# ai4ce/SNAC

Hardware: AMD Instinct MI355X
Metric: env-steps/sec at N=65536 envs (2D dynamic dense); bit-exact vs CPU (higher is better)
Workload: dtype f64; 1 GPU; 2D dynamic dense, 65536 envs/GPU, 600 vector steps/pass, uniform random actions (counter RNG), auto-reset, f64 obs of every step written; envs_per_gpu=65536, vector_steps_per_pass=600, env_steps_per_pass=39321600, parallelism=env-shard x1

## Files before the change

include/snac_hip.h:

```cpp
#ifndef SNAC_HIP_H
#define SNAC_HIP_H
#include <stddef.h>
#include <stdint.h>

#ifdef __cplusplus
extern "C" {
#endif

#define SNAC_ABI_VERSION 12

typedef enum snac_status {
    SNAC_OK = 0,
    SNAC_ERR_ARG = -1,
    SNAC_ERR_HIP = -2,
    SNAC_ERR_UNSUPPORTED = -3
} snac_status;

enum { SNAC_ENV_1D = 1, SNAC_ENV_2D = 2, SNAC_ENV_3D = 3 };
enum { SNAC_OBS_F64 = 0, SNAC_OBS_F32 = 1 };
enum { SNAC_OBS_NONE = 0, SNAC_OBS_ALL = 1, SNAC_OBS_LAST = 2, SNAC_OBS_TILED = 3 };
enum { SNAC_FLAG_NEED_RESET = 1 };
enum { SNAC_RULE_BRICK_GT = 1, SNAC_RULE_TIME_GT = 2 };
enum { SNAC_SCALARS_DEFAULT = 0, SNAC_SCALARS_RAW = 1, SNAC_SCALARS_NORM = 2 };
enum { SNAC_TAIL_POSITION = 1, SNAC_TAIL_PLAN = 2, SNAC_TAIL_RECORD = 4 };
// ... 104 lines not shown
typedef struct snac_rollout_record {
    int8_t* actions;
    int8_t* step_size;
    int16_t* plan_idx;
    uint8_t* first;
} snac_rollout_record;
int snac_rollout_rec(const snac_env_desc* desc, const snac_state* st, int32_t T, uint32_t t0, const int8_t* actions,
                     const int8_t* step_size, int obs_mode, void* obs, float* reward, uint8_t* done,
                     const snac_rollout_record* rec, void* stream);

int snac_rollout_tiled(const snac_env_desc* desc, const snac_state* st, int32_t T, uint32_t t0, const int8_t* actions,
                       const int8_t* step_size, int32_t ring_ticks, int32_t first_tick, void* obs, float* reward, uint8_t* done,
                       const snac_rollout_record* rec, void* stream);

int snac_replay_gather(const snac_env_desc* desc, const snac_state* st, int32_t cap, const void* obs_ring,
                       const uint8_t* first_ring, const int16_t* plan_idx_ring, const int32_t* tick_idx,
                       const int32_t* env_idx, int32_t batch, float* s_out, float* s_next_out, float* plan_out,
                       void* stream);
int snac_replay_gather_tiled(const snac_env_desc* desc, const snac_state* st, int32_t cap, const void* obs_ring,
                             const uint8_t* first_ring, const int16_t* plan_idx_ring, const int32_t* tick_idx,
                             const int32_t* env_idx, int32_t batch, float* s_out, float* s_next_out, float* plan_out,
                             void* stream);

int snac_make_plans(const snac_env_desc* desc, const snac_state* st, int32_t first, int32_t count, int32_t sparse,
                    uint64_t seed, int64_t plan_id_base, const int8_t* vertices, int32_t* area_out, void* stream);

int snac_plans_from_grids(const snac_env_desc* desc, const snac_state* st, int32_t m, int32_t first, const snac_state* src,
                          int32_t src_envs, const int32_t* src_rows, const double* environment_memory,
                          const int32_t* total_brick, void* stream);

int snac_observe(const snac_env_desc* desc, const snac_state* st, void* obs, void* stream);

int snac_iou(const snac_env_desc* desc, const snac_state* st, double* out, void* stream);

int snac_export_grid(const snac_env_desc* desc, const snac_state* st, double* out, void* stream);

typedef struct snac_mailbox snac_mailbox;
int snac_mailbox_create(const snac_env_desc* desc, uint32_t idle_us, snac_mailbox** out);
double* snac_mailbox_row(snac_mailbox* mb);
int snac_mailbox_touch(snac_mailbox* mb);
int snac_mailbox_step(snac_mailbox* mb, const snac_env_desc* desc, const snac_state* st, int32_t action, int32_t step_size);
int snac_mailbox_step_n(snac_mailbox* mb, const snac_env_desc* desc, const snac_state* st, const int8_t* actions, const int8_t* step_size);
float* snac_mailbox_reward(snac_mailbox* mb);
uint8_t* snac_mailbox_done(snac_mailbox* mb);
int snac_mailbox_settle(snac_mailbox* mb);
int snac_mailbox_quit(snac_mailbox* mb);
int snac_mailbox_destroy(snac_mailbox* mb);
int snac_mailbox_stats(const snac_mailbox* mb, uint32_t out[8]);

int snac_transition(const snac_env_desc* desc, const snac_state* st, int32_t m, const int32_t* src_index,
                    const int32_t* dst_index, uint32_t t, const int8_t* actions, const int8_t* step_size, void* obs,
                    float* reward, uint8_t* done, void* stream);

typedef struct snac_node2d {
    snac_env_hdr hdr;
    int32_t episode;
    int32_t zero0[3];
    uint32_t board[20];
    uint32_t zero1[4];
} snac_node2d;
int snac_nodes2d_pack(const snac_env_desc* desc, const snac_state* st, const int32_t* rows, int32_t m, snac_node2d* nodes, int32_t pool_rows,
                      const int32_t* node_rows, void* stream);
int snac_nodes2d_unpack(const snac_env_desc* desc, const snac_node2d* nodes, int32_t pool_rows, const int32_t* node_rows, int32_t m, snac_state* st,
                        const int32_t* rows, void* stream);
int snac_transition_nodes2d(const snac_env_desc* desc, const snac_state* st, snac_node2d* nodes, int32_t pool_rows, int32_t m,
                            const int32_t* src_index, const int32_t* dst_index, uint32_t t, const int8_t* actions, const int8_t* step_size,
// ... 120 lines not shown
```

snac_amd/_lib.py:

```python
import ctypes as C
import os
import subprocess

import numpy as np

HERE = os.path.dirname(os.path.abspath(__file__))
LIB_PATH = os.environ.get("SNAC_HIP_LIB") or os.path.join(HERE, "libsnac_hip.so")
CSRC = os.path.join(HERE, "csrc")
INCLUDE = os.path.join(os.path.dirname(HERE), "include")

SNAC_OK = 0
ABI_VERSION = 12
ENV_1D, ENV_2D, ENV_3D = 1, 2, 3
OBS_F64, OBS_F32 = 0, 1
OBS_NONE, OBS_ALL, OBS_LAST, OBS_TILED = 0, 1, 2, 3
FLAG_NEED_RESET = 1
RULE_BRICK_GT, RULE_TIME_GT = 1, 2
SCALARS_DEFAULT, SCALARS_RAW, SCALARS_NORM = 0, 1, 2
TAIL_POSITION, TAIL_PLAN, TAIL_RECORD = 1, 2, 4

EXPORTS = ("snac_version", "snac_last_error", "snac_env_sizes", "snac_obs_dim", "snac_reset", "snac_reset_scalar", "snac_step",
           "snac_step_scalar", "snac_rollout",
           "snac_rollout_rec", "snac_replay_gather", "snac_make_plans", "snac_observe", "snac_iou", "snac_export_grid", "snac_transition",
           "snac_import_state", "snac_obs_equal", "snac_discounted_return", "snac_plans_from_grids", "snac_mailbox_create", "snac_mailbox_row", "snac_mailbox_touch", "snac_mailbox_step", "snac_mailbox_step_n", "snac_mailbox_reward", "snac_mailbox_done",
           "snac_mailbox_quit", "snac_mailbox_settle", "snac_mailbox_destroy", "snac_mailbox_stats", "snac_stream_sync", "snac_rollout_tiled", "snac_replay_gather_tiled", "snac_traj_alloc",
           "snac_traj_alloc_ex", "snac_traj_free", "snac_traj_layout", "snac_traj_describe", "snac_traj_reserved_bytes", "snac_last_kernel", "snac_tuning",
           "snac_nodes2d_pack", "snac_nodes2d_unpack", "snac_transition_nodes2d", "snac_nodes1d_pack", "snac_nodes1d_unpack",
           "snac_transition_nodes1d", "snac_nodes3d_pack", "snac_nodes3d_unpack", "snac_transition_nodes3d",
           "snac_evaluate_nodes1d", "snac_evaluate_nodes2d", "snac_evaluate_nodes3d", "snac_action_dist", "snac_uct_select", "snac_uct_backup",
           "snac_uct_advance", "snac_uct_select_paths", "snac_uct_backup_paths", "snac_observe_nodes1d", "snac_observe_nodes2d",
           "snac_observe_nodes3d", "snac_uct_select_puct", "snac_uct_set_priors", "snac_uct_pick_moves", "snac_uct_restart",
           "snac_uct_returns", "snac_uct_select_paths_norm", "snac_uct_select_puct_norm", "snac_uct_backup_paths_norm", "snac_uct_bounds")


class Sizes(C.Structure):
    _fields_ = [(n, C.c_int32) for n in (
        "obs_dim", "num_actions", "total_step", "half_window", "env_height", "env_width", "plan_height", "plan_width",
        "grid_elems", "grid_elem_bytes", "plan_elems", "plan_elem_bytes")]


class EnvDesc(C.Structure):
    _fields_ = [("kind", C.c_int32), ("dynamic", C.c_int32), ("num_envs", C.c_int32), ("num_plans", C.c_int32),
                ("obs_dtype", C.c_int32), ("static_plan", C.c_int32), ("seed", C.c_uint64), ("env_id_base", C.c_int64),
                ("total_step", C.c_int32), ("rules", C.c_int32), ("frame_value", C.c_int32), ("obs_scalars", C.c_int32),
                ("obs_tail", C.c_int32), ("action_dist", C.c_int32)]


class RolloutRecord(C.Structure):
    _fields_ = [("actions", C.c_void_p), ("step_size", C.c_void_p), ("plan_idx", C.c_void_p), ("first", C.c_void_p)]


class State(C.Structure):
    _fields_ = [("hdr", C.c_void_p), ("episode", C.c_void_p), ("grid", C.c_void_p), ("plans", C.c_void_p),
                ("plan_tb", C.c_void_p), ("stat_episodes", C.c_void_p), ("stat_return", C.c_void_p),
                ("stat_iou_fx", C.c_void_p)]


TRAJ_INFO_WINDOWS = 64


class TrajInfo(C.Structure):
    _fields_ = ([(n, C.c_int32) for n in ("layout", "rebuilds", "pool_groups", "probe_launches", "windows", "windows_slow")]
                + [(n, C.c_float) for n in ("self_us_per_gib", "fast_us_per_gib", "slow_us_per_gib", "window_max_us_per_gib",
                                            "window_mean_us_per_gib", "block_us_per_gib", "build_ms")]
                + [("bytes", C.c_uint64), ("window_us", C.c_float * TRAJ_INFO_WINDOWS)])
# ... 26 lines not shown


def lib():
    global _lib
    if _lib is None:
        if not os.path.exists(LIB_PATH):
            raise SnacError("libsnac_hip.so is not built (%s); run __graft_entry__.build() or `make -C snac_amd/csrc`. "
                            "There is no CPU fallback." % LIB_PATH)
        import torch

        L = C.CDLL(LIB_PATH)
        vp = C.c_void_p
        L.snac_version.restype = C.c_int
        L.snac_last_error.restype = C.c_char_p
        L.snac_last_kernel.restype = C.c_char_p
        L.snac_stream_sync.argtypes = [vp]
        L.snac_env_sizes.argtypes = [C.c_int, C.c_int, C.POINTER(Sizes)]
        L.snac_obs_dim.argtypes = [C.POINTER(EnvDesc)]
        L.snac_reset.argtypes = [C.POINTER(EnvDesc), C.POINTER(State), vp, vp, vp, vp]
        L.snac_reset_scalar.argtypes = [C.POINTER(EnvDesc), C.POINTER(State), C.c_int32, vp, vp]
        L.snac_step_scalar.argtypes = [C.POINTER(EnvDesc), C.POINTER(State), C.c_uint32, C.c_int32, C.c_int32, C.c_int, vp, vp, vp, vp]
        L.snac_step.argtypes = [C.POINTER(EnvDesc), C.POINTER(State), C.c_uint32, vp, vp, C.c_int, vp, vp, vp, vp]
        L.snac_rollout.argtypes = [C.POINTER(EnvDesc), C.POINTER(State), C.c_int32, C.c_uint32, vp, vp, C.c_int, vp, vp, vp, vp]
        L.snac_rollout_rec.argtypes = [C.POINTER(EnvDesc), C.POINTER(State), C.c_int32, C.c_uint32, vp, vp, C.c_int, vp, vp, vp,
                                       C.POINTER(RolloutRecord), vp]
        L.snac_replay_gather.argtypes = [C.POINTER(EnvDesc), C.POINTER(State), C.c_int32, vp, vp, vp, vp, vp, C.c_int32, vp, vp, vp, vp]
        L.snac_replay_gather_tiled.argtypes = L.snac_replay_gather.argtypes
        L.snac_rollout_tiled.argtypes = [C.POINTER(EnvDesc), C.POINTER(State), C.c_int32, C.c_uint32, vp, vp, C.c_int32, C.c_int32, vp, vp, vp,
                                         C.POINTER(RolloutRecord), vp]
        L.snac_make_plans.argtypes = [C.POINTER(EnvDesc), C.POINTER(State), C.c_int32, C.c_int32, C.c_int32, C.c_uint64, C.c_int64, vp, vp, vp]
        L.snac_observe.argtypes = [C.POINTER(EnvDesc), C.POINTER(State), vp, vp]
        L.snac_iou.argtypes = [C.POINTER(EnvDesc), C.POINTER(State), vp, vp]
        L.snac_export_grid.argtypes = [C.POINTER(EnvDesc), C.POINTER(State), vp, vp]
        L.snac_transition.argtypes = [C.POINTER(EnvDesc), C.POINTER(State), C.c_int32, vp, vp, C.c_uint32, vp, vp, vp, vp, vp, vp]
        L.snac_nodes2d_pack.argtypes = [C.POINTER(EnvDesc), C.POINTER(State), vp, C.c_int32, vp, C.c_int32, vp, vp]
        L.snac_nodes2d_unpack.argtypes = [C.POINTER(EnvDesc), vp, C.c_int32, vp, C.c_int32, C.POINTER(State), vp, vp]
        L.snac_transition_nodes2d.argtypes = [C.POINTER(EnvDesc), C.POINTER(State), vp, C.c_int32, C.c_int32, vp, vp, C.c_uint32, vp, vp, vp, vp, vp, vp]
        for k in ("1d", "3d"):
            getattr(L, "snac_nodes%s_pack" % k).argtypes = L.snac_nodes2d_pack.argtypes
            getattr(L, "snac_nodes%s_unpack" % k).argtypes = L.snac_nodes2d_unpack.argtypes
            getattr(L, "snac_transition_nodes%s" % k).argtypes = L.snac_transition_nodes2d.argtypes
        L.snac_import_state.argtypes = [C.POINTER(EnvDesc), C.POINTER(State), C.c_int32, vp, vp, vp, vp, vp, vp, vp, vp]
        L.snac_plans_from_grids.argtypes = [C.POINTER(EnvDesc), C.POINTER(State), C.c_int32, C.c_int32, C.POINTER(State), C.c_int32, vp, vp, vp, vp]
        L.snac_mailbox_create.argtypes = [C.POINTER(EnvDesc), C.c_uint32, C.POINTER(vp)]
        L.snac_mailbox_row.argtypes, L.snac_mailbox_row.restype = [vp], vp
        L.snac_mailbox_reward.argtypes, L.snac_mailbox_reward.restype = [vp], vp
        L.snac_mailbox_done.argtypes, L.snac_mailbox_done.restype = [vp], vp
        L.snac_mailbox_step_n.argtypes = [vp, C.POINTER(EnvDesc), C.POINTER(State), vp, vp]
        L.snac_mailbox_touch.argtypes = [vp]
        L.snac_mailbox_step.argtypes = [vp, C.POINTER(EnvDesc), C.POINTER(State), C.c_int32, C.c_int32]
        L.snac_mailbox_quit.argtypes = [vp]
        L.snac_mailbox_settle.argtypes = [vp]
        L.snac_mailbox_destroy.argtypes = [vp]
        L.snac_mailbox_stats.argtypes = [vp, C.POINTER(C.c_uint32 * 8)]
        L.snac_obs_equal.argtypes = [C.POINTER(EnvDesc), vp, vp, C.c_int32, vp, vp, C.c_int32, C.c_int32, vp, vp]
        L.snac_discounted_return.argtypes = [C.c_int32, C.c_int32, vp, vp, vp, vp, vp, vp, vp]
        for k in ("1d", "2d", "3d"):
            getattr(L, "snac_evaluate_nodes%s" % k).argtypes = [C.POINTER(EnvDesc), C.POINTER(State), vp, C.c_int32, C.c_int32, vp, C.c_int32, C.c_uint32,
                                                                vp, vp, vp, vp]
        L.snac_action_dist.argtypes = [C.c_int32, C.POINTER(C.c_uint32), C.POINTER(C.c_int32)]
        L.snac_uct_select.argtypes = [C.c_int32, vp, C.c_int32, C.c_int32, C.c_int32, C.c_double, vp, vp, C.c_int32, vp, vp, vp, vp, vp, vp, vp, vp]
        L.snac_uct_backup.argtypes = [C.c_int32, vp, C.c_int32, C.c_int32, C.c_int32, C.c_double, vp, vp, vp, vp, vp, vp, vp, vp]
        L.snac_uct_advance.argtypes = [C.c_int32, vp, C.c_int32, C.c_int32, C.c_int32, vp, C.c_int32, C.c_int32, vp, vp, vp, vp, vp, vp, vp, vp]
        L.snac_uct_select_paths.argtypes = [C.c_int32, vp, C.c_int32, C.c_int32, C.c_int32, C.c_int32, C.c_double, C.c_double, vp, vp, C.c_int32,
                                            vp, vp, vp, vp, vp, vp, vp, vp, vp]
        L.snac_uct_backup_paths.argtypes = [C.c_int32, vp, C.c_int32, C.c_int32, C.c_int32, C.c_int32, C.c_double, vp, vp, vp, vp, vp, vp, vp, vp]
# ... 68 lines not shown
```

snac_amd/batched.py:

```python
import ctypes as C

import numpy as np
import torch

from . import _lib
from . import plans as _plans

_KINDS = {1: 1, 2: 2, 3: 3, "1d": 1, "2d": 2, "3d": 3, "1D": 1, "2D": 2, "3D": 3}
_GRID_DTYPE = {1: torch.int16, 2: torch.int32, 3: torch.int16}


def _ptr(t):
    return None if t is None else C.c_void_p(t.data_ptr())


_raw_stream = getattr(torch._C, "_cuda_getCurrentRawStream", None)
_current_device = getattr(torch._C, "_cuda_getDevice", None) or torch.cuda.current_device


def _meta(*tensors):
    return tuple(None if t is None else (t.shape, t.stride(), t.dtype) for t in tensors)


class BatchedDMPEnv:

    LAYOUTS = {None: {}, "lnet1d": dict(obs_tail=("position",)), "lnet2d": dict(frame_value=2, obs_scalars="norm"),
               "ppo": dict(obs_scalars="raw"), "ppo_plan": dict(obs_scalars="raw", obs_tail=("plan",))}
    _TAILS = {"position": _lib.TAIL_POSITION, "plan": _lib.TAIL_PLAN, "record": _lib.TAIL_RECORD}

    def __init__(self, kind, dynamic, num_envs, plans=None, plan_choose=0, density="dense", split="train",
                 device="cuda", seed=1, obs_dtype=torch.float64, env_id_base=0, total_step=None, plan_tb=None,
                 brick_gt=False, time_gt=False, layout=None, frame_value=None, obs_scalars=None, obs_tail=None, static_plan=0,
                 empty_plans=None, action_probs=None):
# ... 28 lines not shown
        if not isinstance(tail, int):
            tail = sum(self._TAILS[t] for t in set(tail))
        self.obs_tail = int(tail)
        self.total_step = int(total_step) if total_step else sz.total_step
        dev, N = self.device, self.num_envs
        if empty_plans is not None:
            P = int(empty_plans)
            if plans is not None or not 1 <= P <= 32767:
                raise ValueError("empty_plans: 1 .. 32767 rows, without `plans`")
            self.num_plans = P
            self.plans_full = None
            self._plans_stale = True
            self._plans = torch.zeros((P, sz.plan_elems), dtype=torch.int32 if self.kind == 2 else torch.int16, device=dev)
            self._plan_tb = torch.ones((P,), dtype=torch.int16, device=dev)
        else:
            if plans is None:
                if self.dynamic:
                    plans = _plans.dataset(self.kind, density, split)
                else:
                    plans = _plans.static_plan(self.kind, plan_choose)[None]
            self.plans_full = np.array(plans, np.float64)
            packed, tb = _plans.pack_plans(self.kind, self.plans_full)
            if plan_tb is not None:
                tb = np.asarray(plan_tb).astype(np.int16)
                if tb.shape != (len(packed),) or tb.min() < 1:
                    raise ValueError("plan_tb must hold one positive total_brick per plan")
            self.num_plans = len(packed)
            self._plans = torch.from_numpy(packed.view(np.int32) if self.kind == 2 else packed).to(dev)
            self._plan_tb = torch.from_numpy(tb).to(dev)
        self._hdr = torch.zeros((N, 4), dtype=torch.int32, device=dev)
        self._episode = torch.full((N,), -1, dtype=torch.int32, device=dev)
        self._grid = torch.zeros((N, sz.grid_elems), dtype=_GRID_DTYPE[self.kind], device=dev)
        self._stats = torch.zeros((3, N), dtype=torch.int64, device=dev)
        self._desc = _lib.EnvDesc(self.kind, int(self.dynamic), N, self.num_plans,
                                  _lib.OBS_F64 if obs_dtype == torch.float64 else _lib.OBS_F32, int(static_plan),
                                  self.seed & 0xFFFFFFFFFFFFFFFF, self.env_id_base, self.total_step,
                                  (_lib.RULE_BRICK_GT if brick_gt else 0) | (_lib.RULE_TIME_GT if time_gt else 0),
                                  self.frame_value,
                                  {None: _lib.SCALARS_DEFAULT, "raw": _lib.SCALARS_RAW, "norm": _lib.SCALARS_NORM}[self.obs_scalars],
                                  self.obs_tail, 0)
        self.set_action_probs(action_probs)
        self.obs_dim = self._lib.snac_obs_dim(C.byref(self._desc))
        if self.obs_dim < 0:
            _lib.check(self.obs_dim)
        self.base_obs_dim = sz.obs_dim
        self.brick_gt, self.time_gt = bool(brick_gt), bool(time_gt)
        self.static_plan = int(static_plan)
        self._state = _lib.State(self._hdr.data_ptr(), self._episode.data_ptr(), self._grid.data_ptr(),
                                 self._plans.data_ptr(), self._plan_tb.data_ptr(), self._stats[0].data_ptr(),
                                 self._stats[1].data_ptr(), self._stats[2].data_ptr())
        self.t = 0
        self._was_reset = False
        self._fast = None
        self._table_version, self._table_snapshot = 0, None
        self._dev_index = self.device.index
        self._desc_ref, self._state_ref = C.byref(self._desc), C.byref(self._state)
        self._snac_step = self._lib.snac_step
        self._snac_step_scalar, self._snac_sync = self._lib.snac_step_scalar, self._lib.snac_stream_sync
        self._ssf = None
        self._host_ok = None
        self._mapped = {}
        self._mb, self._mb_dirty, self._mb_final = None, False, None

    def set_action_probs(self, action_probs):
        if action_probs is None:
            self._action_weights, self.action_probs, self.action_cdf = None, None, None
            self._desc.action_dist = 0
            return
        cdf = _lib.action_cdf(action_probs, self.num_actions)
        handle = _lib.action_dist(self.num_actions, cdf)
        w = np.array(action_probs, dtype=np.float64)
        self._action_weights, self.action_probs, self.action_cdf = w, w / w.sum(), cdf
        self._desc.action_dist = handle

    def _settle(self):
        if self._mb is not None:
            rc = self._lib.snac_mailbox_settle(self._mb)
            if rc:
                _lib.check(rc)

    def _stream(self):
        if self._mb is not None:
            self._settle()
            self._mb_dirty = True
        raw = getattr(torch._C, "_cuda_getCurrentRawStream", None)
        if raw is not None:
            return C.c_void_p(raw(self.device.index))
        return C.c_void_p(torch.cuda.current_stream(self.device).cuda_stream)

    def _is_mapped(self, t):
        if t.device.type != "cpu":
            return False
        if self._mapped.get(id(t)) is t:
            return True
        if not t.is_pinned():
            return False
        if len(self._mapped) >= 32:
            self._mapped.clear()
        self._mapped[id(t)] = t
        return True

    def _i8(self, x, shape, what):
        if x is None:
            return None
        if torch.is_tensor(x) and x.dtype == torch.int8 and x.is_contiguous() and tuple(x.shape) == tuple(shape) \
                and (x.device == self.device or self._is_mapped(x)):
            return x
        if not torch.is_tensor(x):
            x = torch.as_tensor(np.asarray(x), device=self.device)
        if x.device != self.device:
            x = x.to(self.device)
        if tuple(x.shape) != tuple(shape):
            raise ValueError("%s must have shape %s, got %s" % (what, tuple(shape), tuple(x.shape)))
        return x.to(torch.int8).contiguous()

    def _new_obs(self, *lead):
        return torch.empty(tuple(lead) + (self.num_envs, self.obs_dim), dtype=self.obs_dtype, device=self.device)
# ... 604 lines not shown

    @property
    def count_step(self):
        return self._h16()[:, 3].to(torch.int64)

    @property
    def total_brick(self):
        return self._h16()[:, 4].to(torch.int64)

    @property
    def plan_idx(self):
        return self._h16()[:, 5].to(torch.int64)

    @property
    def episode_return(self):
        return self._h16()[:, 6].to(torch.int64)

    @property
    def episode(self):
        self._settle()
        return self._episode.to(torch.int64)

    def plan(self):
        self._sync_plans_full()
        table = torch.from_numpy(self.plans_full).to(self.device)
        return table[self.plan_idx]

    def input_plan(self):
        if self.kind == 1:
            return self.plan()
        return self.plan()[:, 3:23, 3:23]

    def episodic_stats(self):
        self._settle()
        s = self._stats.sum(dim=1).tolist()
        return dict(episodes=int(s[0]), return_sum=int(s[1]), iou_fx_sum=int(s[2]))

    def stats_tensor(self, out=None):
        self._settle()
        if out is None:
            return self._stats.sum(dim=1)
        return torch.sum(self._stats, dim=1, out=out)
```

snac_amd/csrc/k_roll2d.hip:

```cpp
#include "snac_dev.h"

namespace {



template <bool DYN, typename OT, int WPB, bool EXPL, bool VAR>
__global__ __launch_bounds__(WPB * 64) void k_rollout2d(const KArgs a) {
    using K = K2D<DYN, 64>;
    constexpr int E = 64, D = K::D, RS = K::RS, GE = K::GE;
    constexpr int IMG_WORDS = 26 * RS * 2;
    constexpr int PL_WORDS = (GE * 65 + 3) & ~3;
    constexpr int CMP_WORDS = VAR ? E * VAR_CMP_WORDS : 0;
    constexpr int STG_WORDS = (VAR ? VAR_STG_BYTES : TILE_STG_BYTES) / 4;
    constexpr int WAVE_WORDS = IMG_WORDS + STG_WORDS + PL_WORDS + CMP_WORDS;
    static_assert(IMG_WORDS % 4 == 0 && WAVE_WORDS % 4 == 0, "16-byte aligned staging tiles");
    __shared__ __attribute__((aligned(16))) uint32_t lds_all[WPB * WAVE_WORDS];
    const int lane = threadIdx.x & 63, wv = (int)(threadIdx.x >> 6);
    const int tile = (int)blockIdx.x * WPB + wv;
    const int env0 = __builtin_amdgcn_readfirstlane(tile * E);
    if (env0 >= a.n) return;
    const int nenv = min(E, a.n - env0);
    const bool active = lane < nenv;
    const int env = env0 + (active ? lane : 0);
    uint32_t* const lds = lds_all + wv * WAVE_WORDS;
    uint64_t* const cells = K::cells(lds);
    char* const stg = (char*)(lds + IMG_WORDS);
    uint32_t* const pl = lds + IMG_WORDS + STG_WORDS;
    Lane s;
    s.clear();
    s.r = 3; s.c = 3;
    int episode = 0;
    if (active) { s.unpack(a.hdr[env]); episode = a.episode[env]; }
    K::load_grid(lds, a, env0, nenv, lane);
    const uint64_t gid = (uint64_t)(a.env_id_base + env);
    const EnvKeys sk = env_keys(a.key_step, gid), pk = env_keys(a.key_plan, gid);
    int pcnt = 0, gcnt = 0, inter = 0;
    {
        const uint32_t* const prow = (const uint32_t*)a.plans + (size_t)s.pidx * GE;
        for (int q = 0; q < GE; ++q) {
            const uint32_t p = prow[q];
            pl[q * 65 + lane] = p; pcnt += __popc(p);
            const uint32_t g = active ? K::decode_row(cells[(q + 3) * RS + lane]) : 0u;
            gcnt += __popc(g); inter += __popc(g & p);
        }
    }
    double dtb = (double)s.tb, rtb = 1.0 / dtb;
    const double dT = (double)a.total_step, rT = 1.0 / dT;
    int d_eps = 0, d_ret = 0;
    long long d_iou = 0;
    const bool tl = a.obs_mode == SNAC_OBS_TILED;
    const int LD = VAR ? a.ld : D;
    char* const obs0 = (char*)a.obs + (tl ? (((size_t)(env0 >> 6) * (size_t)a.tiled_T + (size_t)a.tiled_t0) * 64 + (size_t)(env0 & 63)) * LD : (size_t)env0 * LD) * sizeof(OT);
    const size_t tstride = (tl ? (size_t)64 * LD : (size_t)a.n * LD) * sizeof(OT);
    int na = 0, nk = 1;
    if constexpr (EXPL) {
        if (active && a.actions) na = (int)a.actions[(size_t)env0 + lane];
        if (active && a.step_size) nk = (int)a.step_size[(size_t)env0 + lane];
    }
    for (int t = 0; t < a.T; ++t) {
        const size_t row = (size_t)t * (size_t)a.n + (size_t)env0;
        const bool nr = active && a.auto_reset && (s.flags & SNAC_FLAG_NEED_RESET);
        if (__builtin_expect(__any(nr), 0)) {
            bool fresh = false;
            if (nr) {
                const int old_pidx = s.pidx;
                episode += 1;
                const int pidx = pick_plan<K>(a, pk, episode, old_pidx);
                if (pidx != old_pidx) { fresh = true; s.pidx = pidx; }
                s.r = 3; s.c = 3; s.cb = 0; s.cs = 0; s.ep_ret = 0; s.cross = 0; s.flags = 0;
                gcnt = 0; inter = 0;
            }
            for (unsigned long long m = __ballot(nr); m; m &= m - 1) K::clear(lds, __ffsll(m) - 1, lane);
            for (unsigned long long m = __ballot(fresh); m; m &= m - 1) {
                const int e = __ffsll(m) - 1;
                const int pe = __builtin_amdgcn_readlane(s.pidx, e);
                cmem_u32* const src = (cmem_u32*)(uintptr_t)a.plans + (size_t)pe * GE;
                cmem_u32* const tbw = (cmem_u32*)(uintptr_t)a.plan_tb + (pe >> 1);
                uint32_t rw[GE];
// ... 66 lines not shown
            if (__builtin_expect(__any(active && s.tb <= 0), 0)) {
                asm volatile("" ::: "memory");
                v0 = c0 / dtb;
            }
        }
        if constexpr (VAR) {
            const int recv[8] = {reward, done ? 1 : 0, s.r, s.c, s.cb, s.cs, s.tb, s.pidx};
            emit_rows_var<OT>(stg, pl + PL_WORDS, obs0 + (size_t)t * tstride, lane, nenv, LD, a.tail, a.frame_val, wr, v0, v1, recv,
                              [&](int e, int row) { return pl[row * 65 + e]; });
        } else {
            emit_tile<OT, sizeof(OT) == 4>(stg, obs0 + (size_t)t * tstride, lane, nenv,
                          [&](int el) { const int i = el / 7, j = el - 7 * i; return ((int)(wr[i] << (30 - 2 * j))) >> 30; },
                          v0, v1);
        }
    }
    K::store_grid(lds, a, env0, nenv, lane);
    if (active) {
        a.hdr[env] = s.pack();
        a.episode[env] = episode;
        if (d_eps) {
            a.stat_episodes[env] += d_eps;
            a.stat_return[env] += d_ret;
            a.stat_iou_fx[env] += d_iou;
        }
    }
}


template <bool DYN, typename OT>
void launch_roll2d_w(const KArgs& a, hipStream_t s) {
    const int tiles = (a.n + 63) / 64;
    const dim3 grid((unsigned)((tiles + 3) / 4)), block(256);
    const bool expl = a.actions || a.step_size;
    if (a.variant) {
        if (expl) hipLaunchKernelGGL((k_rollout2d<DYN, OT, 4, true, true>), grid, block, 0, s, a);
        else hipLaunchKernelGGL((k_rollout2d<DYN, OT, 4, false, true>), grid, block, 0, s, a);
    } else {
        if (expl) hipLaunchKernelGGL((k_rollout2d<DYN, OT, 4, true, false>), grid, block, 0, s, a);
        else hipLaunchKernelGGL((k_rollout2d<DYN, OT, 4, false, false>), grid, block, 0, s, a);
    }
}

}

namespace snac_detail {

void launch_roll2d(const snac_env_desc* d, const KArgs& a, hipStream_t s) {
    const bool dyn = d->dynamic != 0, f32 = d->obs_dtype == SNAC_OBS_F32;
    if (dyn) f32 ? launch_roll2d_w<true, float>(a, s) : launch_roll2d_w<true, double>(a, s);
    else f32 ? launch_roll2d_w<false, float>(a, s) : launch_roll2d_w<false, double>(a, s);
}

}
```

snac_amd/csrc/snac_hip.hip:

```cpp
#include "snac_dev.h"

#include <atomic>

namespace snac_detail {
void launch_step3dq(const snac_env_desc* d, const KArgs& a, hipStream_t s);
void launch_step1d(const snac_env_desc* d, const KArgs& a, hipStream_t s);
void launch_edges1d(const snac_env_desc* d, const KArgs& a, hipStream_t s);
void launch_reset(const snac_env_desc* d, const KArgs& a, hipStream_t s);
void launch_iou(const snac_env_desc* d, const KArgs& a, hipStream_t s);
void launch_aux1d(const snac_env_desc* d, const KArgs& a, hipStream_t s);
void launch_aux2d(const snac_env_desc* d, const KArgs& a, hipStream_t s);
void launch_aux3d(const snac_env_desc* d, const KArgs& a, hipStream_t s);
void launch_roll2db(const snac_env_desc* d, const KArgs& a, int steppers, hipStream_t s);
void launch_roll2dbv(const snac_env_desc* d, const KArgs& a, int steppers, hipStream_t s);
void launch_roll3dbv(const snac_env_desc* d, const KArgs& a, hipStream_t s);
thread_local char g_err[256] = "";
thread_local const char* g_kernel = "";

struct ActDist { int32_t num_actions; uint32_t cdf[7]; };
constexpr int ACT_DIST_CAP = 1024;
ActDist g_dists[ACT_DIST_CAP];
std::atomic<int> g_ndists{0};
std::mutex g_dists_mu;

// ... 128 lines not shown
     {"SNAC_STEP3D_QUARTER_MAX", 1 << 30, "... up to this many (524 288: 67.5 against k_step3ds' 76.6 us, 131 072: 23.9 / 23.6)"},
     {"SNAC_1D_TP_EB8_MIN", 3584, "k_rollout1dt blocks hold 8 envs from this many envs (two blocks share a CU: one computes its chunk while the other's rows leave; 4096 envs: 0.045 against 0.048 ms on 16-env blocks, 32 768: 0.351 / 0.421, 65 536: 0.685 / 0.920; r06_1d.txt) ..."},
     {"SNAC_1D_TP_EB8_MAX", 1 << 30, "... up to this many"},
     {"SNAC_STEP3D_NTLOAD_MIN", 376832, "k_step3dq from this many envs on: non-temporal span loads + plain row stores; below, where state and rows fit the Infinity Cache: plain span loads (the state stays cached) + non-temporal row stores (65 536 envs: 12.9 -> 10.5 us per tick, 131 072: 24.1 -> 19.1; 262 144: 39.6 against 41.3 / 43.5 the other way, 524 288: 71 against 101; r06_step_loads.txt)"},
     {"SNAC_STEP3D_HUGE_MIN", 557056, "k_step3dq from this many envs on (the rows of one tick alone overflow the Infinity Cache): the form SNAC_STEP3D_HUGE_FORM"},
     {"SNAC_STEP3D_HUGE_FORM", 3, "bit 0: non-temporal span loads, bit 1: non-temporal row stores (655 360 envs: 135 us per tick with 1, 109 with 2, 99 with 3; 1 048 576: 237 / 160 / 157)"},
     {"SNAC_STEP3D_FORM", -1, "k_step3dq: force a form (bits as above) whatever the batch size; -1: by batch size"},
     {"SNAC_STEP2D_PLAIN_LO", 20480, "k_step2d reads its records with PLAIN loads from this many envs (below: non-temporal loads, plain rows: 16 384 envs 6.5 against 6.8 us) ..."},
     {"SNAC_STEP2D_RES_HI", 278528, "k_step2d inside SNAC_STEP2D_PLAIN_LO .. this many envs also stores its rows NON-TEMPORALLY (the resident form: 32 768 envs 7.9 -> 6.8 us per tick, 65 536: 8.4 -> 7.7-7.8, 262 144: 22.6 -> 22.3; 294 912: 24.7 against 24.9, 458 752: 37.0 against 39.7)"},
     {"SNAC_STEP2D_PLAIN_HI", 475136, "... up to this many, with non-temporal loads outside (81 920 envs: 10.6 -> 10.4 us, 262 144: 26.5 -> 22.7, 458 752: 41.5 -> 37.0; 65 536: 8.4 against 8.75 plain, 524 288: 46.5 against 49.4)"},
     {"SNAC_STEP2D_HUGE_MIN", 475137, "k_step2d from this many envs on: the form SNAC_STEP2D_HUGE_FORM (the 2D state of a million envs is 105 MB: it fits the Infinity Cache at every batch size, the rows of a tick do not)"},
     {"SNAC_STEP2D_HUGE_FORM", 2, "bit 0: non-temporal record loads, bit 1: non-temporal row stores (524 288 envs: 46.4 us per tick with 1, 43.5 with 2; 1 048 576: 146 / 82; r06_step_loads.txt)"},
     {"SNAC_STEP2D_FORM", -1, "k_step2d, canonical rows: force a form (bits as above) whatever the batch size; -1: by batch size"},
     {"SNAC_NODES2D_NT", 1, "k_edges2dp (2D edges on node records): 1 = the observation rows leave as NON-TEMPORAL stores -- streamed rows then do not displace the node records in the Infinity Cache (65.1 -> 50.3 us per 524 288 edges of a 2^20-record pool, r06_edges.txt)"},
     {"SNAC_1D_LANE", 1, "1D rollouts of large batches on k_rollout1dl (lane = env; canonical rows, every row written, N % 4 == 0, aligned obs) ..."},
     {"SNAC_1D_LANE_MIN_F64", 45056, "... float64 rows from this many envs (a wave of 64 envs per SIMD at 65 536: 0.454 ms per 750 ticks = 6.6 TB/s against 0.69-0.73 on the time-parallel kernel; 45 056: 7.5e10 env-steps/s against 6.7e10, 40 960: 6.7 against 6.9; r06_1d_lane.txt) ..."},
     {"SNAC_1D_LANE_MIN_F32", 36864, "... float32 rows from this many (the lane kernel: 0.37 ms per 750 ticks whatever the batch up to 65 536 envs; the time-parallel one by box: 36 864 envs 0.35-0.42 ms, 40 960 0.39-0.49, 32 768 0.31-0.39; r06_1d_lane.txt, r06_retune_1d.txt)"},
     {"SNAC_1D_LANE_NT", 0, "k_rollout1dl: 1 = its rows leave as non-temporal stores (65 536 envs: 0.468 against 0.454 ms with float64 rows, level with float32: off)"},
     {"SNAC_STEP1D", 1, "the canonical 1D snac_step on identity rows (N % 4 == 0, aligned obs) on k_step1d: 64 envs per wave, wide loads, the rows as one run per wave (0 = the tile kernel k_transition) ..."},
     {"SNAC_STEP1D_MIN", 256, "... from this many envs"},
     {"SNAC_STEP1D_FORM", 2, "k_step1d: bit 0 = its records by non-temporal loads, bit 1 = its rows by non-temporal stores.  Records and rows of every batch size fit the Infinity Cache: the resident form (2) at 524 288 envs 15.5 us per tick, both plain 16.2, non-temporal loads 18.4-18.9 (r06_step1d.txt)"},
     {"SNAC_EDGES1D", 1, "1D tree edges with gathered rows (snac_transition with index arrays, canonical layout) on k_edges1d: the records through LDS, four lanes per record (0 = the tile kernel k_transition) ..."},
     {"SNAC_EDGES1D_MIN", 64, "... from this many edges per call"},
     {"SNAC_STEP1D_VAR_MIN", 256, "k_step1d takes the 1D layout variants (rows of 8 .. 46 values) from this many envs (1024 envs with the 37-value PPO rows: 5.4 against 6.5 us per tick on the tile kernel, 65 536: 6.9 / 23.0, 524 288 with 8-value L-Net rows: 18.3 / 44.1; r06_step1d.txt)"},
     {"SNAC_1D_LANE_VAR_MIN", 28672, "k_rollout1dl takes the 1D layout variants with rows of more than 16 values from this many envs (37-value PPO rows: 1.75 ms per 750 ticks up to 32 768 envs, 2.19 at 65 536 = 6.8 TB/s; k_rollout1dt's VAR form 1.01 / 2.07 / 4.21 ms at 16 384 / 32 768 / 65 536; r06_1d_lane.txt) ..."},
     {"SNAC_1D_LANE_VAR_SHORT_MIN", 49152, "... and those with rows of at most 16 values from this many (8-value L-Net rows: 0.78 ms flat; k_rollout1dt 0.76 at 45 056, 1.05 at 65 536)"},
     {"SNAC_RESET_FAST", 1, "snac_reset / snac_reset_scalar of every env (no mask), canonical layout, N % 4 == 0, aligned obs, on k_reset: nothing of the old state is read but the episode counter; records zeroed and rows written as runs (0 = the tile kernel k_aux) ..."},
     {"SNAC_RESET_FAST_MIN", 256, "... from this many envs"},
     {"SNAC_IOU_FAST", 1, "snac_iou on k_iou (lane = env, no LDS; 3D: the header alone) from 256 envs; 0 = the tile kernel k_aux, which loads every record into LDS first"},
     {"SNAC_AUX_STEP", 1, "snac_reset with a mask and snac_observe (canonical layout, N % 4 == 0, aligned obs, from 256 envs) on the step kernels' AUX forms (k_step1d / k_step2d / k_step3dq without a step); 0 = the tile kernel k_aux"},
     {"SNAC_EVAL_E", 64, "leaves per wave of k_eval for 1D / 2D leaves (snac_evaluate_nodes1d / 2d; 16 / 32 / 64): 2D, 65 536 leaves, H = 600: 0.320 against 0.359 ms per call with 32, 4096 leaves level (0.275 / 0.274); 1D, 65 536 leaves, H = 300: 0.172 / 0.194 (r08_eval.txt)"},
     {"SNAC_EVAL3D_E", 16, "leaves per wave of k_eval for 3D leaves (16 / 32 / 64: 22 / 44 / 88 KB of LDS per wave): 65 536 leaves, H = 200: 0.219 ms per call against 0.262 with 32 and 0.355 with 64; 4096 leaves: 0.142 / 0.166 / 0.160 (r08_eval.txt)"},
     {"SNAC_UCT_BOUNDS_WIDTH", 0, "lanes per tree of k_uct_bounds (snac_uct_bounds; 8 / 16 / 32 / 64): 0 = from cap, 8 lanes up to 32 nodes per tree, 16 up to 64, 32 up to 128, a wave above (r15_uct_norm.txt)"},
};

int tune(int id) {
    static int v[TN_COUNT];
    static std::once_flag once;
    std::call_once(once, [] {
        for (int i = 0; i < TN_COUNT; ++i) { const char* e = std::getenv(KNOBS[i].env); v[i] = e ? std::atoi(e) : KNOBS[i].def; }
    });
    return v[id];
}

int pick_tile(int kind, int n) {
    const int forced = tune(TN_TILE);
    if (kind == SNAC_ENV_3D) return forced == 16 ? 16 : 8;
    if (forced == 8 || forced == 16 || forced == 32 || forced == 64) return forced;
    const int shift = kind == SNAC_ENV_1D ? 1 : 0;
    if (n >= (64 * 1024) << shift) return 64;
    if (n >= (32 * 1024) << shift) return 32;
    if (n >= (16 * 1024) << shift) return 16;
    return 8;
}

bool pipeline_off() { return tune(TN_PIPELINE) == 0; }
inline bool every_row(const KArgs& a) { return a.obs_mode == SNAC_OBS_ALL || a.obs_mode == SNAC_OBS_TILED; }
inline bool pieces16(const KArgs& a) { return (a.n & 3) == 0 && (((uintptr_t)a.obs) & 15) == 0; }

bool roll3db_ok(const KArgs& a, bool f32) {
    const int lim = tune(TN_3D_BLOCK_MIN) >= 0 ? tune(TN_3D_BLOCK_MIN) : tune(f32 ? TN_3D_BLOCK_MIN_F32 : TN_3D_BLOCK_MIN_F64);
    if (a.variant) {
        const int from = (a.tail & SNAC_TAIL_PLAN) ? tune(f32 ? TN_3D_BLOCK_VAR_PLAN_F32 : TN_3D_BLOCK_VAR_PLAN_F64) : tune(TN_3D_BLOCK_VAR_MIN);
        if (tune(TN_3D_BLOCK_VAR) == 0 || a.n < from || (((uintptr_t)a.plans) & 15) != 0) return false;
        return tune(TN_3D_BLOCK) != 0 && every_row(a) && a.num_plans <= TB_MAX && pieces16(a) && !pipeline_off();
    }
// ... 302 lines not shown
```

snac_amd/csrc/snac_tune.h:

```cpp
#pragma once

namespace snac_detail {
enum Tn { TN_PIPELINE, TN_TILE, TN_2D_TILE32_MIN, TN_3D_BLOCK, TN_3D_BLOCK_MIN, TN_3D_BLOCK_MIN_F64, TN_3D_BLOCK_MIN_F32, TN_2D_STAGE, TN_2D_STAGE_MIN, TN_2D_STAGE_MIN_F64,
          TN_2D_STAGE_MIN_F32, TN_2D_TP, TN_2D_TP_MAX, TN_2D_TP_MAX_F64, TN_2D_TP_GAP_LO, TN_2D_TP_GAP_HI, TN_2D_TP_MAX_F32, TN_2D_TP_MAX_ODD, TN_2D_TP_VAR_MAX,
          TN_2D_TP_VAR_PLAN, TN_2D_TP_VAR_SHORT, TN_2D_TP_EB8, TN_1D_TP, TN_1D_TP_MAX, TN_1D_TP_MAX_F64, TN_1D_TP_MAX_F32, TN_1D_TP_VAR_MAX, TN_1D_TP_EB16,
          TN_STEP_STAGE, TN_STEP_VAR_MIN, TN_STEP_VAR_SHORT, TN_STEP_VAR_HALF_LO, TN_STEP_VAR_HALF_HI, TN_STEP_VAR_F64, TN_STEP_VAR_F32, TN_STEP_VAR_HALF,
          TN_STEP_VAR3_MIN, TN_STEP3D_SPAN, TN_STEP3D_SPAN_MIN, TN_T2D_E, TN_EDGES3D, TN_EDGES2D, TN_EDGES2D_MIN, TN_3D_BLOCK_VAR, TN_3D_BLOCK_VAR_MIN, TN_3D_BLOCK_VAR_PLAN_F64, TN_3D_BLOCK_VAR_PLAN_F32, TN_2D_BLOCK, TN_2D_BLOCK_MIN_F64, TN_2D_BLOCK_MAX_F64, TN_2D_BLOCK_MIN_F32,
          TN_2D_BLOCK_MAX_F32, TN_2D_BLOCK_TWO_F64, TN_2D_BLOCK_TWO_F32, TN_2D_BLOCK_VAR_MIN, TN_2D_BLOCK_VAR_MAX, TN_2D_BLOCK_VAR_TWO, TN_2D_BLOCK_FOUR_F64, TN_2D_BLOCK_FOUR_F32, TN_STEP3D_QUARTER, TN_STEP3D_QUARTER_MIN, TN_STEP3D_QUARTER_MAX, TN_1D_TP_EB8_MIN, TN_1D_TP_EB8_MAX, TN_STEP3D_NTLOAD_MIN, TN_STEP3D_HUGE_MIN, TN_STEP3D_HUGE_FORM, TN_STEP3D_FORM, TN_STEP2D_PLAIN_LO, TN_STEP2D_RES_HI, TN_STEP2D_PLAIN_HI, TN_STEP2D_HUGE_MIN, TN_STEP2D_HUGE_FORM, TN_STEP2D_FORM, TN_NODES2D_NT, TN_1D_LANE, TN_1D_LANE_MIN_F64, TN_1D_LANE_MIN_F32, TN_1D_LANE_NT, TN_STEP1D, TN_STEP1D_MIN, TN_STEP1D_FORM, TN_EDGES1D, TN_EDGES1D_MIN, TN_STEP1D_VAR_MIN, TN_1D_LANE_VAR_MIN, TN_1D_LANE_VAR_SHORT_MIN, TN_RESET_FAST, TN_RESET_FAST_MIN, TN_IOU_FAST, TN_AUX_STEP, TN_EVAL_E, TN_EVAL3D_E, TN_UCT_BOUNDS_WIDTH, TN_COUNT };
int tune(int id);

}
```

Measured before the change: 16.94 billion env-steps/s.

## Load 2D rollout head with 16-byte pieces and add native stats-sum kernel

The 2D rollout kernel's prologue now loads the header, board grid and plan row as 16-byte vector pieces in two dependent stages, replacing one-dword loops that chain many dependent memory round trips. The path is enabled by default when the grid and plan pointers are 16-byte aligned. Separately, a single-pass stats reduction kernel with a ticket-based last-block finish replaces the torch sum in stats_tensor. The wide head holds more registers per lane, which may reduce occupancy.

```diff
diff --git a/include/snac_hip.h b/include/snac_hip.h
--- a/include/snac_hip.h
+++ b/include/snac_hip.h
@@ -160,6 +160,9 @@
 int snac_observe(const snac_env_desc* desc, const snac_state* st, void* obs, void* stream);
 
 int snac_iou(const snac_env_desc* desc, const snac_state* st, double* out, void* stream);
+
+#define SNAC_STATS_SCRATCH_BYTES 4096
+int snac_stats_sum(const snac_state* st, int32_t n, int64_t* out, void* scratch, void* stream);
 
 int snac_export_grid(const snac_env_desc* desc, const snac_state* st, double* out, void* stream);
 
diff --git a/snac_amd/_lib.py b/snac_amd/_lib.py
--- a/snac_amd/_lib.py
+++ b/snac_amd/_lib.py
@@ -18,6 +18,7 @@
 RULE_BRICK_GT, RULE_TIME_GT = 1, 2
 SCALARS_DEFAULT, SCALARS_RAW, SCALARS_NORM = 0, 1, 2
 TAIL_POSITION, TAIL_PLAN, TAIL_RECORD = 1, 2, 4
+STATS_SCRATCH_BYTES = 4096
 
 EXPORTS = ("snac_version", "snac_last_error", "snac_env_sizes", "snac_obs_dim", "snac_reset", "snac_reset_scalar", "snac_step",
            "snac_step_scalar", "snac_rollout",
@@ -30,7 +31,7 @@
            "snac_evaluate_nodes1d", "snac_evaluate_nodes2d", "snac_evaluate_nodes3d", "snac_action_dist", "snac_uct_select", "snac_uct_backup",
            "snac_uct_advance", "snac_uct_select_paths", "snac_uct_backup_paths", "snac_observe_nodes1d", "snac_observe_nodes2d",
            "snac_observe_nodes3d", "snac_uct_select_puct", "snac_uct_set_priors", "snac_uct_pick_moves", "snac_uct_restart",
-           "snac_uct_returns", "snac_uct_select_paths_norm", "snac_uct_select_puct_norm", "snac_uct_backup_paths_norm", "snac_uct_bounds")
+           "snac_uct_returns", "snac_uct_select_paths_norm", "snac_uct_select_puct_norm", "snac_uct_backup_paths_norm", "snac_uct_bounds", "snac_stats_sum")
 
 
 class Sizes(C.Structure):
@@ -123,6 +124,7 @@
         L.snac_observe.argtypes = [C.POINTER(EnvDesc), C.POINTER(State), vp, vp]
         L.snac_iou.argtypes = [C.POINTER(EnvDesc), C.POINTER(State), vp, vp]
         L.snac_export_grid.argtypes = [C.POINTER(EnvDesc), C.POINTER(State), vp, vp]
+        L.snac_stats_sum.argtypes = [C.POINTER(State), C.c_int32, vp, vp, vp]
         L.snac_transition.argtypes = [C.POINTER(EnvDesc), C.POINTER(State), C.c_int32, vp, vp, C.c_uint32, vp, vp, vp, vp, vp, vp]
         L.snac_nodes2d_pack.argtypes = [C.POINTER(EnvDesc), C.POINTER(State), vp, C.c_int32, vp, C.c_int32, vp, vp]
         L.snac_nodes2d_unpack.argtypes = [C.POINTER(EnvDesc), vp, C.c_int32, vp, C.c_int32, C.POINTER(State), vp, vp]
diff --git a/snac_amd/batched.py b/snac_amd/batched.py
--- a/snac_amd/batched.py
+++ b/snac_amd/batched.py
@@ -1,4 +1,5 @@
 import ctypes as C
+import os
 
 import numpy as np
 import torch
@@ -93,6 +94,8 @@
         self._episode = torch.full((N,), -1, dtype=torch.int32, device=dev)
         self._grid = torch.zeros((N, sz.grid_elems), dtype=_GRID_DTYPE[self.kind], device=dev)
         self._stats = torch.zeros((3, N), dtype=torch.int64, device=dev)
+        self._stats_scratch = torch.zeros((_lib.STATS_SCRATCH_BYTES // 8,), dtype=torch.int64, device=dev)
+        self._stats_native = os.environ.get("SNAC_STATS_NATIVE", "1") != "0"
         self._desc = _lib.EnvDesc(self.kind, int(self.dynamic), N, self.num_plans,
                                   _lib.OBS_F64 if obs_dtype == torch.float64 else _lib.OBS_F32, int(static_plan),
                                   self.seed & 0xFFFFFFFFFFFFFFFF, self.env_id_base, self.total_step,
@@ -144,6 +147,9 @@
         if self._mb is not None:
             self._settle()
             self._mb_dirty = True
+        return self._stream_ro()
+
+    def _stream_ro(self):
         raw = getattr(torch._C, "_cuda_getCurrentRawStream", None)
         if raw is not None:
             return C.c_void_p(raw(self.device.index))
@@ -814,12 +820,17 @@
         return self.plan()[:, 3:23, 3:23]
 
     def episodic_stats(self):
-        self._settle()
-        s = self._stats.sum(dim=1).tolist()
+        s = self.stats_tensor().tolist()
         return dict(episodes=int(s[0]), return_sum=int(s[1]), iou_fx_sum=int(s[2]))
 
     def stats_tensor(self, out=None):
         self._settle()
+        if out is not None and not (out.dtype == torch.int64 and tuple(out.shape) == (3,) and out.device == self.device and out.is_contiguous()):
+            return torch.sum(self._stats, dim=1, out=out)
+        if not self._stats_native:
+            return self._stats.sum(dim=1) if out is None else torch.sum(self._stats, dim=1, out=out)
         if out is None:
-            return self._stats.sum(dim=1)
-        return torch.sum(self._stats, dim=1, out=out)
+            out = torch.empty((3,), dtype=torch.int64, device=self.device)
+        with torch.cuda.device(self.device):
+            _lib.check(self._lib.snac_stats_sum(self._state_ref, self.num_envs, _ptr(out), _ptr(self._stats_scratch), self._stream_ro()))
+        return out
diff --git a/snac_amd/csrc/k_roll2d.hip b/snac_amd/csrc/k_roll2d.hip
--- a/snac_amd/csrc/k_roll2d.hip
+++ b/snac_amd/csrc/k_roll2d.hip
@@ -4,7 +4,7 @@
 
 
 
-template <bool DYN, typename OT, int WPB, bool EXPL, bool VAR>
+template <bool DYN, typename OT, int WPB, bool EXPL, bool VAR, bool WIDE>
 __global__ __launch_bounds__(WPB * 64) void k_rollout2d(const KArgs a) {
     using K = K2D<DYN, 64>;
     constexpr int E = 64, D = K::D, RS = K::RS, GE = K::GE;
@@ -30,12 +30,43 @@
     s.clear();
     s.r = 3; s.c = 3;
     int episode = 0;
-    if (active) { s.unpack(a.hdr[env]); episode = a.episode[env]; }
-    K::load_grid(lds, a, env0, nenv, lane);
-    const uint64_t gid = (uint64_t)(a.env_id_base + env);
-    const EnvKeys sk = env_keys(a.key_step, gid), pk = env_keys(a.key_plan, gid);
     int pcnt = 0, gcnt = 0, inter = 0;
-    {
+    static_assert(GE % 4 == 0 && (E * GE) % (4 * 64) == 0, "the wide head: whole 16-byte pieces, the same number for every lane");
+    constexpr int PIECES = GE / 4;
+    if constexpr (WIDE) {
+        const uint4* const gsrc = (const uint4*)((const uint32_t*)a.grid + (size_t)env0 * GE) + lane;
+        const int npieces = nenv * PIECES;
+        int4 h = make_int4(0, 0, 0, 0);
+        if (active) h = a.hdr[env];
+        uint4 gw[PIECES];
+#pragma unroll
+        for (int j = 0; j < PIECES; ++j) { gw[j] = make_uint4(0u, 0u, 0u, 0u); if (j * 64 + lane < npieces) gw[j] = gsrc[j * 64]; }
+        if (active) { episode = a.episode[env]; s.unpack(h); }
+        const uint4* const psrc = (const uint4*)((const uint32_t*)a.plans + (size_t)s.pidx * GE);
+        uint4 pw[PIECES];
+#pragma unroll
+        for (int j = 0; j < PIECES; ++j) pw[j] = psrc[j];
+        for (int i = lane; i < 3 * RS; i += 64) { cells[i] = 0x000FFFFFFFFFFFFFull; cells[23 * RS + i] = 0x000FFFFFFFFFFFFFull; }
+#pragma unroll
+        for (int j = 0; j < PIECES; ++j) {
+            const int p = j * 64 + lane, e = p / PIECES, row = (p - e * PIECES) * 4;
+            uint64_t* const c = cells + (row + 3) * RS + e;
+            if (p < npieces) { c[0] = K::encode_row(gw[j].x); c[RS] = K::encode_row(gw[j].y); c[2 * RS] = K::encode_row(gw[j].z); c[3 * RS] = K::encode_row(gw[j].w); }
+        }
+#pragma unroll
+        for (int j = 0; j < PIECES; ++j) {
+            const uint32_t p4[4] = {pw[j].x, pw[j].y, pw[j].z, pw[j].w};
+#pragma unroll
+            for (int k = 0; k < 4; ++k) {
+                const int q = 4 * j + k;
+                pl[q * 65 + lane] = p4[k]; pcnt += __popc(p4[k]);
+                const uint32_t g = active ? K::decode_row(cells[(q + 3) * RS + lane]) : 0u;
+                gcnt += __popc(g); inter += __popc(g & p4[k]);
+            }
+        }
+    } else {
+        if (active) { s.unpack(a.hdr[env]); episode = a.episode[env]; }
+        K::load_grid(lds, a, env0, nenv, lane);
         const uint32_t* const prow = (const uint32_t*)a.plans + (size_t)s.pidx * GE;
         for (int q = 0; q < GE; ++q) {
             const uint32_t p = prow[q];
@@ -44,6 +75,8 @@
             gcnt += __popc(g); inter += __popc(g & p);
         }
     }
+    const uint64_t gid = (uint64_t)(a.env_id_base + env);
+    const EnvKeys sk = env_keys(a.key_step, gid), pk = env_keys(a.key_plan, gid);
     double dtb = (double)s.tb, rtb = 1.0 / dtb;
     const double dT = (double)a.total_step, rT = 1.0 / dT;
     int d_eps = 0, d_ret = 0;
@@ -176,13 +209,16 @@
     const int tiles = (a.n + 63) / 64;
     const dim3 grid((unsigned)((tiles + 3) / 4)), block(256);
     const bool expl = a.actions || a.step_size;
+    const bool wide = snac_detail::tune(snac_detail::TN_2D_WIDE_HEAD) != 0 && (((uintptr_t)a.grid | (uintptr_t)a.plans) & 15) == 0;
+    void (*kern)(const KArgs);
     if (a.variant) {
-        if (expl) hipLaunchKernelGGL((k_rollout2d<DYN, OT, 4, true, true>), grid, block, 0, s, a);
-        else hipLaunchKernelGGL((k_rollout2d<DYN, OT, 4, false, true>), grid, block, 0, s, a);
+        if (expl) kern = wide ? k_rollout2d<DYN, OT, 4, true, true, true> : k_rollout2d<DYN, OT, 4, true, true, false>;
+        else kern = wide ? k_rollout2d<DYN, OT, 4, false, true, true> : k_rollout2d<DYN, OT, 4, false, true, false>;
     } else {
-        if (expl) hipLaunchKernelGGL((k_rollout2d<DYN, OT, 4, true, false>), grid, block, 0, s, a);
-        else hipLaunchKernelGGL((k_rollout2d<DYN, OT, 4, false, false>), grid, block, 0, s, a);
-    }
+        if (expl) kern = wide ? k_rollout2d<DYN, OT, 4, true, false, true> : k_rollout2d<DYN, OT, 4, true, false, false>;
+        else kern = wide ? k_rollout2d<DYN, OT, 4, false, false, true> : k_rollout2d<DYN, OT, 4, false, false, false>;
+    }
+    hipLaunchKernelGGL(kern, grid, block, 0, s, a);
 }
 
 }
diff --git a/snac_amd/csrc/k_stats.hip b/snac_amd/csrc/k_stats.hip
--- /dev/null
+++ b/snac_amd/csrc/k_stats.hip
@@ -0,0 +1,75 @@
+#include "snac_dev.h"
+
+namespace {
+
+constexpr int STATS_BLOCKS = 64, STATS_PER_BLOCK = 2048;
+static_assert((STATS_BLOCKS * 3 + 1) * 8 <= SNAC_STATS_SCRATCH_BYTES, "the scratch holds every workgroup's partial sums and the ticket");
+
+__device__ __forceinline__ long long wave_sum(long long v) {
+    for (int off = 32; off > 0; off >>= 1) v += __shfl_xor(v, off);
+    return v;
+}
+
+__global__ __launch_bounds__(256) void k_stats_sum(const int64_t* __restrict__ s0, const int64_t* __restrict__ s1, const int64_t* __restrict__ s2, const int n,
+                                                   int64_t* __restrict__ out, int64_t* const scratch) {
+    __shared__ long long sh[4 * 3 + 1];
+    const int lane = threadIdx.x & 63, wv = (int)(threadIdx.x >> 6);
+    const long long stride = (long long)gridDim.x * 256;
+    long long i = (long long)blockIdx.x * 256 + threadIdx.x;
+    long long a0 = 0, a1 = 0, a2 = 0;
+    for (; i + 3 * stride < n; i += 4 * stride) {
+        const long long x0 = s0[i], x1 = s0[i + stride], x2 = s0[i + 2 * stride], x3 = s0[i + 3 * stride];
+        const long long y0 = s1[i], y1 = s1[i + stride], y2 = s1[i + 2 * stride], y3 = s1[i + 3 * stride];
+        const long long z0 = s2[i], z1 = s2[i + stride], z2 = s2[i + 2 * stride], z3 = s2[i + 3 * stride];
+        a0 += (x0 + x1) + (x2 + x3); a1 += (y0 + y1) + (y2 + y3); a2 += (z0 + z1) + (z2 + z3);
+    }
+    for (; i < n; i += stride) { a0 += s0[i]; a1 += s1[i]; a2 += s2[i]; }
+    a0 = wave_sum(a0); a1 = wave_sum(a1); a2 = wave_sum(a2);
+    if (lane == 0) { sh[wv * 3] = a0; sh[wv * 3 + 1] = a1; sh[wv * 3 + 2] = a2; }
+    __syncthreads();
+    unsigned int* const ticket = (unsigned int*)(scratch + STATS_BLOCKS * 3);
+    if (threadIdx.x == 0) {
+        int64_t* const mine = scratch + (size_t)blockIdx.x * 3;
+        for (int k = 0; k < 3; ++k)
+            __hip_atomic_store(mine + k, (int64_t)(sh[k] + sh[3 + k] + sh[6 + k] + sh[9 + k]), __ATOMIC_RELAXED, __HIP_MEMORY_SCOPE_AGENT);
+        __builtin_amdgcn_fence(__ATOMIC_RELEASE, "agent");
+        asm volatile("s_waitcnt vmcnt(0)" ::: "memory");
+        const unsigned int t = __hip_atomic_fetch_add(ticket, 1u, __ATOMIC_RELAXED, __HIP_MEMORY_SCOPE_AGENT);
+        sh[12] = t == gridDim.x - 1 ? 1 : 0;
+    }
+    __syncthreads();
+    if (sh[12] == 0 || wv != 0) return;
+    __builtin_amdgcn_fence(__ATOMIC_ACQUIRE, "agent");
+    asm volatile("s_waitcnt vmcnt(0)" ::: "memory");
+    long long t0 = 0, t1 = 0, t2 = 0;
+    for (int b = lane; b < (int)gridDim.x; b += 64) {
+        t0 += __hip_atomic_load(scratch + b * 3, __ATOMIC_RELAXED, __HIP_MEMORY_SCOPE_AGENT);
+        t1 += __hip_atomic_load(scratch + b * 3 + 1, __ATOMIC_RELAXED, __HIP_MEMORY_SCOPE_AGENT);
+        t2 += __hip_atomic_load(scratch + b * 3 + 2, __ATOMIC_RELAXED, __HIP_MEMORY_SCOPE_AGENT);
+    }
+    t0 = wave_sum(t0); t1 = wave_sum(t1); t2 = wave_sum(t2);
+    if (lane == 0) {
+        out[0] = t0; out[1] = t1; out[2] = t2;
+        __hip_atomic_store(ticket, 0u, __ATOMIC_RELAXED, __HIP_MEMORY_SCOPE_AGENT);
+    }
+}
+
+}
+
+extern "C" {
+
+int snac_stats_sum(const snac_state* st, int32_t n, int64_t* out, void* scratch, void* stream) {
+    if (!st || !st->stat_episodes || !st->stat_return || !st->stat_iou_fx) return fail(SNAC_ERR_ARG, "null pointer in snac_state");
+    if (n < 1) return fail(SNAC_ERR_ARG, "n must be >= 1");
+    if (!out || !scratch) return fail(SNAC_ERR_ARG, "null out / scratch");
+    if ((((uintptr_t)out | (uintptr_t)scratch | (uintptr_t)st->stat_episodes | (uintptr_t)st->stat_return | (uintptr_t)st->stat_iou_fx) & 7) != 0)
+        return fail(SNAC_ERR_ARG, "the sums, out and scratch must be 8-byte aligned");
+    const int blocks = std::min(STATS_BLOCKS, (int)(((int64_t)n + STATS_PER_BLOCK - 1) / STATS_PER_BLOCK));
+    hipLaunchKernelGGL(k_stats_sum, dim3((unsigned)blocks), dim3(256), 0, (hipStream_t)stream, (const int64_t*)st->stat_episodes,
+                       (const int64_t*)st->stat_return, (const int64_t*)st->stat_iou_fx, (int)n, out, (int64_t*)scratch);
+    const hipError_t e = hipGetLastError();
+    if (e != hipSuccess) return fail_hip(e, "stats sum launch");
+    return SNAC_OK;
+}
+
+}
diff --git a/snac_amd/csrc/snac_hip.hip b/snac_amd/csrc/snac_hip.hip
--- a/snac_amd/csrc/snac_hip.hip
+++ b/snac_amd/csrc/snac_hip.hip
@@ -184,6 +184,7 @@
      {"SNAC_EVAL_E", 64, "leaves per wave of k_eval for 1D / 2D leaves (snac_evaluate_nodes1d / 2d; 16 / 32 / 64): 2D, 65 536 leaves, H = 600: 0.320 against 0.359 ms per call with 32, 4096 leaves level (0.275 / 0.274); 1D, 65 536 leaves, H = 300: 0.172 / 0.194 (r08_eval.txt)"},
      {"SNAC_EVAL3D_E", 16, "leaves per wave of k_eval for 3D leaves (16 / 32 / 64: 22 / 44 / 88 KB of LDS per wave): 65 536 leaves, H = 200: 0.219 ms per call against 0.262 with 32 and 0.355 with 64; 4096 leaves: 0.142 / 0.166 / 0.160 (r08_eval.txt)"},
      {"SNAC_UCT_BOUNDS_WIDTH", 0, "lanes per tree of k_uct_bounds (snac_uct_bounds; 8 / 16 / 32 / 64): 0 = from cap, 8 lanes up to 32 nodes per tree, 16 up to 64, 32 up to 128, a wave above (r15_uct_norm.txt)"},
+     {"SNAC_2D_WIDE_HEAD", 1, "k_rollout2d: full tiles with a 16-byte aligned grid and plan table load header, boards and plan row as 16-byte pieces in two dependent stages; 0 = the one-dword loops (K2D::load_grid + the plan-row loop, ~41 dependent round trips per launch; profiles/rollout2d_head_stats_sum.txt)"},
 };
 
 int tune(int id) {
diff --git a/snac_amd/csrc/snac_tune.h b/snac_amd/csrc/snac_tune.h
--- a/snac_amd/csrc/snac_tune.h
+++ b/snac_amd/csrc/snac_tune.h
@@ -6,7 +6,7 @@
           TN_2D_TP_VAR_PLAN, TN_2D_TP_VAR_SHORT, TN_2D_TP_EB8, TN_1D_TP, TN_1D_TP_MAX, TN_1D_TP_MAX_F64, TN_1D_TP_MAX_F32, TN_1D_TP_VAR_MAX, TN_1D_TP_EB16,
           TN_STEP_STAGE, TN_STEP_VAR_MIN, TN_STEP_VAR_SHORT, TN_STEP_VAR_HALF_LO, TN_STEP_VAR_HALF_HI, TN_STEP_VAR_F64, TN_STEP_VAR_F32, TN_STEP_VAR_HALF,
           TN_STEP_VAR3_MIN, TN_STEP3D_SPAN, TN_STEP3D_SPAN_MIN, TN_T2D_E, TN_EDGES3D, TN_EDGES2D, TN_EDGES2D_MIN, TN_3D_BLOCK_VAR, TN_3D_BLOCK_VAR_MIN, TN_3D_BLOCK_VAR_PLAN_F64, TN_3D_BLOCK_VAR_PLAN_F32, TN_2D_BLOCK, TN_2D_BLOCK_MIN_F64, TN_2D_BLOCK_MAX_F64, TN_2D_BLOCK_MIN_F32,
-          TN_2D_BLOCK_MAX_F32, TN_2D_BLOCK_TWO_F64, TN_2D_BLOCK_TWO_F32, TN_2D_BLOCK_VAR_MIN, TN_2D_BLOCK_VAR_MAX, TN_2D_BLOCK_VAR_TWO, TN_2D_BLOCK_FOUR_F64, TN_2D_BLOCK_FOUR_F32, TN_STEP3D_QUARTER, TN_STEP3D_QUARTER_MIN, TN_STEP3D_QUARTER_MAX, TN_1D_TP_EB8_MIN, TN_1D_TP_EB8_MAX, TN_STEP3D_NTLOAD_MIN, TN_STEP3D_HUGE_MIN, TN_STEP3D_HUGE_FORM, TN_STEP3D_FORM, TN_STEP2D_PLAIN_LO, TN_STEP2D_RES_HI, TN_STEP2D_PLAIN_HI, TN_STEP2D_HUGE_MIN, TN_STEP2D_HUGE_FORM, TN_STEP2D_FORM, TN_NODES2D_NT, TN_1D_LANE, TN_1D_LANE_MIN_F64, TN_1D_LANE_MIN_F32, TN_1D_LANE_NT, TN_STEP1D, TN_STEP1D_MIN, TN_STEP1D_FORM, TN_EDGES1D, TN_EDGES1D_MIN, TN_STEP1D_VAR_MIN, TN_1D_LANE_VAR_MIN, TN_1D_LANE_VAR_SHORT_MIN, TN_RESET_FAST, TN_RESET_FAST_MIN, TN_IOU_FAST, TN_AUX_STEP, TN_EVAL_E, TN_EVAL3D_E, TN_UCT_BOUNDS_WIDTH, TN_COUNT };
+          TN_2D_BLOCK_MAX_F32, TN_2D_BLOCK_TWO_F64, TN_2D_BLOCK_TWO_F32, TN_2D_BLOCK_VAR_MIN, TN_2D_BLOCK_VAR_MAX, TN_2D_BLOCK_VAR_TWO, TN_2D_BLOCK_FOUR_F64, TN_2D_BLOCK_FOUR_F32, TN_STEP3D_QUARTER, TN_STEP3D_QUARTER_MIN, TN_STEP3D_QUARTER_MAX, TN_1D_TP_EB8_MIN, TN_1D_TP_EB8_MAX, TN_STEP3D_NTLOAD_MIN, TN_STEP3D_HUGE_MIN, TN_STEP3D_HUGE_FORM, TN_STEP3D_FORM, TN_STEP2D_PLAIN_LO, TN_STEP2D_RES_HI, TN_STEP2D_PLAIN_HI, TN_STEP2D_HUGE_MIN, TN_STEP2D_HUGE_FORM, TN_STEP2D_FORM, TN_NODES2D_NT, TN_1D_LANE, TN_1D_LANE_MIN_F64, TN_1D_LANE_MIN_F32, TN_1D_LANE_NT, TN_STEP1D, TN_STEP1D_MIN, TN_STEP1D_FORM, TN_EDGES1D, TN_EDGES1D_MIN, TN_STEP1D_VAR_MIN, TN_1D_LANE_VAR_MIN, TN_1D_LANE_VAR_SHORT_MIN, TN_RESET_FAST, TN_RESET_FAST_MIN, TN_IOU_FAST, TN_AUX_STEP, TN_EVAL_E, TN_EVAL3D_E, TN_UCT_BOUNDS_WIDTH, TN_2D_WIDE_HEAD, TN_COUNT };
 int tune(int id);
 
 }
```

Measured after the change: 17.09 billion env-steps/s, median of 6. Within noise of the previous version (+0.9%).
